# xyy7/Learning-based-RGB-D-Image-Compression

Measured on AMD Instinct MI355X. Metric: RGB-D Mpixels/s encode+decode, higher is better.
Workload: dtype f32; 1 GPU; c3_4x480x640; codec=ELIC_united ch4 q=2_2 (N=192,M=320), images_per_gpu=4, steps_per_call=4, images_per_call=16, calls=5, weights=synthetic seed 0 (stress recipe), streams=per image, y_bytes_last_batch=15943588, engine_instances=5, conv_tiles=throughput, warmup_steps_run=40, launch=HIP graph per call shape, pairs_in_flight=80

## Files before the change

include/rgbd_amd.h:

```cpp
#ifndef RGBD_AMD_H
#define RGBD_AMD_H

#include <stddef.h>
#include <stdint.h>

#ifdef __cplusplus
extern "C" {
#endif

#define RGBD_AMD_ABI_VERSION 1

int rgbd_abi_version(void);

int rgbd_set_blocking_sync(int32_t on);
int rgbd_get_blocking_sync(void);

int rgbd_pmf_to_quantized_cdf(const float* pmf, int32_t n, int32_t precision, uint32_t* cdf_out);

typedef struct rgbd_tables rgbd_tables;

int rgbd_tables_create(const int32_t* cdf, int32_t cdf_stride, const int32_t* cdf_sizes, const int32_t* offsets,
                       int32_t n_cdf, rgbd_tables** out);
void rgbd_tables_destroy(rgbd_tables* t);

// ... 157 lines not shown
int rgbd_elic_debug_floats(rgbd_elic* m, int32_t modality, float* x, float* scale, int64_t cap, int64_t* n);
int rgbd_elic_set_forced_symbols(rgbd_elic* m, int32_t modality, const int32_t* y_sym, int64_t n_y, const int32_t* z_sym,
                                 int64_t n_z);

int rgbd_debug_force_splitk(int32_t s);
int rgbd_debug_force_fuse(int32_t mode);
int rgbd_debug_force_subpix(int32_t mode);
int rgbd_debug_force_pair(int32_t mode);
int rgbd_elic_set_tile_mode(rgbd_elic* m, int32_t mode);
int rgbd_debug_bench_streams(int32_t n);
int rgbd_debug_force_blocked(int32_t on);
int rgbd_debug_force_ckbd(int32_t part);
int rgbd_debug_conv_log(int32_t on);
int64_t rgbd_debug_conv_log_read(char* buf, int64_t cap);
int rgbd_debug_force_tile(const char* cfg);
long rgbd_debug_tile_list(int32_t blocked, char* buf, long cap);
int rgbd_debug_tile_override(const char* csv);

int rgbd_pointwise_nchw(int32_t op, const float* x_dev, int32_t n, int32_t c, int32_t h, int32_t w, int32_t oh, int32_t ow,
                        const float* w0, const float* w1, float* y_dev, void* stream);

int rgbd_ref_channel_mean(const float* x_dev, int32_t n, int32_t c, int32_t h, int32_t w, float* mean_dev, int32_t mstride,
                          void* stream);
int rgbd_ref_linear(const float* weight, const float* x_dev, int32_t n, int32_t K, int32_t J, const int32_t* row_class, int32_t form,
                    int32_t act, int32_t stage, float* y_dev, void* stream);
int rgbd_ref_sigmoid_gate(const float* t_dev, const float* mul_dev, const float* res_dev, int32_t n, int32_t c, int32_t h, int32_t w,
                          int32_t per_image, int32_t threads, float* y_dev, void* stream);
int rgbd_ref_small_conv_nchw(const float* x_dev, int32_t n, int32_t cin, int32_t h, int32_t w, const float* weight, const float* bias,
                             int32_t cout, int32_t k, int32_t stride, int32_t pad, int32_t act, int32_t ckbd, const int32_t* kblocks,
                             int32_t nkblocks, const float* res1_dev, const float* mul_dev, const float* res2_dev, float* y_dev,
// ... 47 lines not shown
```

learning-based-rgb-d-image-compression_amd/_lib.py:

```python
import ctypes
import os
import subprocess

_HERE = os.path.dirname(os.path.abspath(__file__))
_SO = os.path.join(_HERE, "librgbd_amd.so")
_SO = os.environ.get("RGBD_AMD_LIB", _SO)
_SRCS = ["conv_mfma.hip", "conv_mfma_blk.hip", "pointwise.hip", "swin.hip", "entropy.hip", "metrics.hip", "coder_abi.hip", "gdn.hip", "engine.hip", "engine_abi.hip"]
_LIB = None

ERRORS = {-22: "invalid argument", -12: "out of memory", -5: "HIP runtime error", -28: "buffer too small",
          -1: "wrong call order / missing weights or tables"}


class RgbdError(RuntimeError):
    pass


def check(rc: int, what: str = ""):
    if rc != 0:
        raise RgbdError(f"librgbd_amd: {what} failed with {rc} ({ERRORS.get(rc, 'unknown')})")


class ConvFormsOps(ctypes.Structure):
    _fields_ = [("x_dev", ctypes.c_void_p)] + [(n, ctypes.POINTER(ctypes.c_float)) for n in
# ... 8 lines not shown
               [(n, ctypes.c_int32) for n in ("cout2", "act_mid", "cout3", "x_off", "x_total", "y_off", "y_total", "y2_off", "y2_total",
                                              "y3_off", "y3_total", "groups")] + \
               [("set", ConvFormsOps * 2)]


def build(force: bool = False, verbose: bool = False) -> str:
    from concurrent.futures import ThreadPoolExecutor

    csrc = os.path.join(_HERE, "csrc")
    objdir = os.path.join(csrc, "build")
    hdrs = [os.path.join(csrc, "common.h"), os.path.join(csrc, "exact_math.h"),
            os.path.join(os.path.dirname(_HERE), "include", "rgbd_amd.h")]
    body, tiles = os.path.join(csrc, "conv_mfma_body.h"), os.path.join(csrc, "conv_tiles.h")
    extra = {"conv_mfma.hip": [body, tiles, os.path.join(csrc, "tile_table.h"), os.path.join(csrc, "tile_table_loaded.h"),
                               os.path.join(csrc, "tile_table_blk.h"), os.path.join(csrc, "tile_table_blk_loaded.h")],
             "conv_mfma_blk.hip": [body, tiles]}
    hdrs.append(os.path.join(csrc, "splitk_table.h"))
    extra["coder_abi.hip"] = extra["gdn.hip"] = [os.path.join(csrc, "engine_internal.h")]
    extra["engine.hip"] = extra["engine_abi.hip"] = [os.path.join(csrc, "engine_internal.h"), os.path.join(csrc, "engine.h"),
                                                     os.path.join(csrc, "conv_args.h")]
    hipcc = os.environ.get("HIPCC", "/opt/rocm/bin/hipcc")
    os.makedirs(objdir, exist_ok=True)
    jobs, objs = [], []
    for name in _SRCS:
        src, obj = os.path.join(csrc, name), os.path.join(objdir, name + ".o")
        objs.append(obj)
        deps = [src] + hdrs + extra.get(name, [])
        if force or not os.path.exists(obj) or any(os.path.getmtime(obj) < os.path.getmtime(d) for d in deps):
            flags = ["-mllvm", "-amdgpu-mfma-vgpr-form"] if name == "conv_mfma_blk.hip" else []
            jobs.append([hipcc, "-O3", "--offload-arch=gfx950", "-ffp-contract=off", "-fPIC", "-std=c++17"] + flags + ["-c", src, "-o", obj])
    if not jobs and os.path.exists(_SO) and all(os.path.getmtime(_SO) >= os.path.getmtime(o) for o in objs):
        return _SO
    if verbose:
        for j in jobs:
            print(" ".join(j))
    with ThreadPoolExecutor(max_workers=4) as ex:
        list(ex.map(subprocess.check_call, jobs))
    subprocess.check_call([hipcc, "--offload-arch=gfx950", "-fPIC", "-shared"] + objs + ["-o", _SO])
    return _SO


def lib():
    global _LIB
    if _LIB is not None:
# ... 101 lines not shown
        "rgbd_debug_force_ckbd": (ctypes.c_int, [c_i32]),
        "rgbd_debug_force_blocked": (ctypes.c_int, [c_i32]),
        "rgbd_debug_force_fuse": (ctypes.c_int, [c_i32]),
        "rgbd_debug_force_subpix": (ctypes.c_int, [c_i32]),
        "rgbd_layernorm": (ctypes.c_int, [c_vp, c_i64, c_i32, c_i32, c_vp, c_vp, c_vp, c_i32, c_vp]),
        "rgbd_debug_force_layernorm_form": (None, [c_i32]),
        "rgbd_layernorm2": (ctypes.c_int, [c_vp, c_i64, c_i32, c_i32, c_vp, c_vp, c_vp, c_i32, c_vp, c_vp, c_vp, c_vp, c_vp]),
        "rgbd_window_attention": (ctypes.c_int, [c_vp] + [c_i32] * 7 + [c_vp, c_vp, c_i32, c_vp, c_vp, c_vp, c_vp]),
        "rgbd_patch_merge_gather": (ctypes.c_int, [c_vp] + [c_i32] * 5 + [c_vp, c_i32, c_vp]),
        "rgbd_pixel_shuffle2": (ctypes.c_int, [c_vp] + [c_i32] * 5 + [c_vp, c_i32, c_vp]),
        "rgbd_debug_force_pair": (ctypes.c_int, [c_i32]),
        "rgbd_debug_fail_captures": (ctypes.c_int, [c_i32]),
        "rgbd_debug_bench_streams": (ctypes.c_int, [c_i32]),
        "rgbd_elic_set_tile_mode": (ctypes.c_int, [ctypes.c_void_p, c_i32]),
        "rgbd_debug_force_tile": (ctypes.c_int, [ctypes.c_char_p]),
        "rgbd_debug_conv_log": (ctypes.c_int, [c_i32]),
        "rgbd_debug_conv_log_read": (c_i64, [ctypes.c_char_p, c_i64]),
        "rgbd_debug_tile_override": (ctypes.c_int, [ctypes.c_char_p]),
        "rgbd_debug_tile_list": (ctypes.c_long, [c_i32, ctypes.c_char_p, ctypes.c_long]),
        "rgbd_conv_bench": (ctypes.c_int, [c_i32] * 11 + [f32p]),
        "rgbd_elic_profile_dump": (ctypes.c_int, [c_vp, ctypes.c_char_p]),
        "rgbd_elic_profile_read": (ctypes.c_int, [c_vp, ctypes.POINTER(ctypes.c_double), i64p,
                                                  ctypes.POINTER(ctypes.c_double)]),
        "rgbd_elic_profile_read_executed": (ctypes.c_int, [c_vp, ctypes.POINTER(ctypes.c_double)]),
    }
    for name, (res, args) in sig.items():
        fn = getattr(L, name)
        fn.restype = res
        fn.argtypes = args
    _LIB = L
    return L


EXPORTS = ["rgbd_abi_version", "rgbd_set_blocking_sync", "rgbd_get_blocking_sync", "rgbd_pmf_to_quantized_cdf", "rgbd_tables_create", "rgbd_tables_destroy",
           "rgbd_rans_max_bytes", "rgbd_rans_encode", "rgbd_rans_decoder_create", "rgbd_rans_decoder_set_stream",
           "rgbd_rans_decoder_decode", "rgbd_rans_decoder_destroy", "rgbd_rans_encode_batch_dev", "rgbd_rans_decode_batch_dev", "rgbd_ckbd_quant_index", "rgbd_ckbd_dequant", "rgbd_conv2d_nchw", "rgbd_conv2d_ref_nchw", "rgbd_conv_forms_nchw", "rgbd_pointwise_nchw", "rgbd_ref_channel_mean", "rgbd_ref_linear", "rgbd_ref_sigmoid_gate",
           "rgbd_ref_small_conv_nchw", "rgbd_ref_deconv_s2_nchw", "rgbd_elic_create",
           "rgbd_elic_destroy", "rgbd_elic_set_ref_blocks", "rgbd_elic_get_refnum", "rgbd_elic_ref_table_misses", "rgbd_elic_clone_shared", "rgbd_elic_set_tensor", "rgbd_elic_set_tables", "rgbd_elic_set_scale_table",
           "rgbd_elic_finalize", "rgbd_elic_compress", "rgbd_elic_forward", "rgbd_elic_stream_count", "rgbd_elic_stream",
           "rgbd_elic_decompress", "rgbd_elic_create_r2d", "rgbd_elic_create_stf", "rgbd_elic_create_single", "rgbd_elic_compress_single", "rgbd_elic_decompress_single", "rgbd_elic_forward_single", "rgbd_elic_compress_united", "rgbd_elic_decompress_united", "rgbd_elic_debug_tensor", "rgbd_elic_debug_symbols", "rgbd_elic_set_debug_floats", "rgbd_elic_debug_floats", "rgbd_elic_set_forced_symbols", "rgbd_elic_set_profile", "rgbd_elic_graph_count", "rgbd_elic_workspace_bytes", "rgbd_msssim_workspace_bytes", "rgbd_msssim_stats", "rgbd_layernorm", "rgbd_debug_force_layernorm_form",
           "rgbd_layernorm2", "rgbd_window_attention", "rgbd_patch_merge_gather", "rgbd_pixel_shuffle2",
           "rgbd_elic_profile_read", "rgbd_elic_profile_read_executed", "rgbd_debug_force_splitk", "rgbd_debug_force_fuse", "rgbd_debug_force_subpix", "rgbd_debug_force_pair", "rgbd_debug_fail_captures", "rgbd_debug_force_ckbd", "rgbd_debug_force_blocked", "rgbd_debug_bench_streams", "rgbd_elic_set_tile_mode", "rgbd_debug_force_tile", "rgbd_debug_conv_log", "rgbd_debug_conv_log_read", "rgbd_debug_tile_override", "rgbd_debug_tile_list", "rgbd_conv_bench",
           "rgbd_elic_profile_dump", "rgbd_elic_create_stf_single", "rgbd_slice_quant_index", "rgbd_slice_dequant", "rgbd_lrp_update",
           "rgbd_ckbd_estimate_part", "rgbd_slice_estimate", "rgbd_ckbd_part", "rgbd_z_quant", "rgbd_z_dequant", "rgbd_eb_forward",
           "rgbd_elic_create_ckbd", "rgbd_gdn_nchw", "rgbd_gdn_parametrize", "rgbd_debug_force_gdn_tile", "rgbd_gdn_bench",
           "rgbd_guided_window_attention", "rgbd_aligner_create", "rgbd_aligner_forward", "rgbd_elic_decompress_single_mid",
           "rgbd_elic_forward_single_mid"]


_BS_HOLDERS = 0


def set_blocking_sync(on: bool) -> bool:
    global _BS_HOLDERS
    import gc

    L = lib()
# ... 9 lines not shown
```

learning-based-rgb-d-image-compression_amd/csrc/common.h:

```cpp
#pragma once
#include <hip/hip_runtime.h>
#include <stdint.h>
#include <stdio.h>

#define RGBD_OK 0
#define RGBD_EINVAL (-22)
#define RGBD_ENOMEM (-12)
#define RGBD_EHIP (-5)
#define RGBD_ENOSPC (-28)
#define RGBD_ESTATE (-1)

#define HIP_TRY(expr)                                                                          \
    do {                                                                                       \
        hipError_t _e = (expr);                                                                \
        if (_e != hipSuccess) {                                                                \
            fprintf(stderr, "[rgbd_amd] %s:%d %s -> %s\n", __FILE__, __LINE__, #expr,          \
                    hipGetErrorString(_e));                                                    \
            return RGBD_EHIP;                                                                  \
        }                                                                                      \
    } while (0)

struct Act {
    float* p = nullptr;
    int n = 0, h = 0, w = 0, c = 0, cs = 0;
// ... 103 lines not shown
    if (nphase == 1 && out_px_per_image <= 512) {
        if (taps_per_phase == 1) s = K >= 1500 ? 8 : (K >= 700 ? 4 : (K >= 350 ? 2 : 1));
        else s = K >= 5000 ? 8 : (K >= 1000 ? 4 : (K >= 500 ? 2 : 1));
    } else {
        s = (int)((K + 800) / 1600);
        if (s > 8) s = 8;
    }
    if (s > cin_pad / 16) s = cin_pad / 16;
    if (s < 1) s = 1;
    return s;
}

int launch_conv(const ConvArgs& a, hipStream_t s);
int conv_fused_plan(int cout_pad, int cout2_pad, int ntaps, int N, int GH, int GW, int loaded);
int launch_conv_fused(const ConvArgs& a, hipStream_t s);
int conv_log_enable(int on);
int conv_tile_override(const char* csv);
long conv_log_read(char* buf, long cap);
long conv_tile_list(int blocked, char* buf, long cap);

int launch_sigmoid_gate_ref(const float* t, int tcs, const float* mul, int mcs, const float* res2, int r2cs, float* y, int ycs,
                            int N, int HW, int C, int per_image, int threads, hipStream_t s);

int launch_nchw_to_nhwc16(const float* src, int N, int C, int H, int W, float* dst, int cs, hipStream_t s, int perm = 0);
int launch_nhwc_to_nchw_clamp(const float* src, int N, int C, int H, int W, int cs, float* dst, int clamp01,
                              hipStream_t s, int perm = 0);
int launch_maxpool7s3(const float* x, int N, int H, int W, int cs, float* y, int OH, int OW, hipStream_t s,
                      const float* x1 = nullptr, float* y1 = nullptr);
int launch_bilinear(const float* x, int N, int h, int w, int cs, float* y, int H, int W, hipStream_t s, const float* x1 = nullptr,
                    float* y1 = nullptr, int ref_channels = 0);
// ... 149 lines not shown
```

learning-based-rgb-d-image-compression_amd/csrc/conv_mfma.hip:

```cpp
#include <array>
#include <map>
#include <string>

#include "conv_mfma_body.h"
#include "conv_tiles.h"

bool conv_blk_tile_ok(int wm, int mt, int nt, int max_tiles);
int launch_conv_blk(const ConvArgs& a, const Choice& c, hipStream_t s);
int launch_conv_fused_blk(const ConvArgs& a, int cls, hipStream_t s);

namespace {

Choice choose(const ConvArgs& a, int max_tiles = 16)
{
    static const int cand[][3] = {{2, 3, 8}, {2, 2, 8}, {2, 5, 4}, {2, 4, 4}, {2, 3, 4}, {2, 2, 4}, {2, 1, 4}, {2, 5, 2}, {2, 4, 2},
                                  {2, 3, 2}, {2, 2, 2}, {2, 1, 2}, {2, 5, 1}, {2, 4, 1}, {2, 3, 1}, {2, 2, 1},
                                  {2, 1, 1}, {1, 3, 2}, {1, 2, 2}, {1, 1, 2}, {1, 3, 1}, {1, 2, 1}, {1, 1, 1}};
    int max_taps = 1;
    for (int p = 0; p < a.nphase; ++p) max_taps = a.taps.n[p] > max_taps ? a.taps.n[p] : max_taps;
    const double K = (double)max_taps * a.cin_pad / a.splitk;
    const int ck = a.ckbd ? 1 : 0;
    const int GWe = ck ? (a.GW + 1) / 2 : a.GW;
    Choice best{2, 4, 4, 16, 4, false};
    double best_cost = -1.0;
// ... 299 lines not shown
    }
    if (t) {
        c.wm = t->wm;
        c.mt = t->mt;
        c.nt = t->nt;
        set_mode(c, t->kc, t->dma);
        c.tw_log2 = pick_tw_log2(a.ckbd ? (a.GW + 1) / 2 : a.GW, a.GH, 16 * t->nt * (t->wm == 2 ? 2 : 4));
    }
    if (g_log_on) {
        char key[160];
        snprintf(key, sizeof(key), "%d,%d,%d,%d,%d,%d,%d,%d,%d", a.N * (a.groups == 2 ? 2 : 1), a.H, a.W, a.cin_pad, a.cout_pad, a.ntaps_total,
                 a.nphase > 1 ? a.OS : a.IS, a.nphase + 10 * a.ckbd + (a.blocked ? 100 : 0), a.splitk);
        std::lock_guard<std::mutex> lk(g_log_mu);
        ++g_log[key];
    }
    if (!g_ovr.empty()) {
        char key[160];
        snprintf(key, sizeof(key), "%d,%d,%d,%d,%d,%d,%d,%d,%d", a.N * (a.groups == 2 ? 2 : 1), a.H, a.W, a.cin_pad, a.cout_pad, a.ntaps_total,
                 a.nphase > 1 ? a.OS : a.IS, a.nphase + 10 * a.ckbd + (a.blocked ? 100 : 0), a.splitk);
        std::lock_guard<std::mutex> lk(g_log_mu);
        auto it = g_ovr.find(key);
        if (it != g_ovr.end()) {
            c.wm = it->second[0];
            c.mt = it->second[1];
            c.nt = it->second[2];
            set_mode(c, it->second[3], it->second[4]);
            c.tw_log2 = pick_tw_log2(a.ckbd ? (a.GW + 1) / 2 : a.GW, a.GH, 16 * c.nt * (c.wm == 2 ? 2 : 4));
        }
    }
    static const char* force_env = getenv("RGBD_CONV_FORCE");
    const char* force = g_conv_force[0] ? g_conv_force : force_env;
    if (force) {
        int wm = c.wm, mt = c.mt, nt = c.nt, kc = c.kc, dm = c.dma;
        sscanf(force, "%d,%d,%d,%d,%d", &wm, &mt, &nt, &kc, &dm);
        c.wm = wm;
        c.mt = mt;
        c.nt = nt;
        set_mode(c, kc, dm);
        c.tw_log2 = pick_tw_log2(a.ckbd ? (a.GW + 1) / 2 : a.GW, a.GH, 16 * nt * (wm == 2 ? 2 : 4));
    }
    static const bool debug = getenv("RGBD_CONV_DEBUG") != nullptr;
    if (debug)
        fprintf(stderr, "[conv] N=%d GH=%d GW=%d cin=%d cout=%d taps=%d IS=%d nph=%d -> WM=%d MT=%d NT=%d KC=%d tw=%d dma=%d\n", a.N,
                a.GH, a.GW, a.cin_pad, a.cout_pad, a.taps.n[0], a.IS, a.nphase, c.wm, c.mt, c.nt, c.kc, 1 << c.tw_log2, (int)c.dma);
    if (c.ring && !ring_ok(a)) return RGBD_ENOSPC;
    if (a.blocked) return launch_conv_blk(a, c, s);
    RGBD_TILES_MAIN_RING(RGBD_RING4)
    RGBD_TILES_MAIN_RING(RGBD_RING3)
    if (c.ring) return RGBD_ENOSPC;
    RGBD_TILES_MAIN(RGBD_CASE)
    return RGBD_EINVAL;
}

static const bool g_fuse_off = getenv("RGBD_NO_FUSE") != nullptr;
int g_fuse_force = -1;
int g_fuse_lead_off = 0;

int conv_fused_plan(int cout_pad, int cout2_pad, int ntaps, int N, int GH, int GW, int loaded)
{
// ... 46 lines not shown
```

learning-based-rgb-d-image-compression_amd/csrc/conv_mfma_body.h:

```cpp
#pragma once
#include <stdlib.h>
#include <string.h>

#include <algorithm>
#include <map>
#include <mutex>
#include <string>

#include "common.h"
#include "exact_math.h"

typedef float f32x4 __attribute__((ext_vector_type(4)));

__device__ __forceinline__ float sigmoid_f32(float x)
{
    return __builtin_amdgcn_rcpf(1.0f + __builtin_amdgcn_exp2f(x * -1.4426950408889634f));
}

template <int N>
__device__ __forceinline__ void rgbd_wait_vmcnt()
{
    asm volatile("s_waitcnt vmcnt(%0)" ::"n"(N) : "memory");
}

template <int WM, int WN, int MT, int NT, int KC, bool DMA, int G2, bool LEAD = false, int NB = 2, bool BLK = false>
__device__ __forceinline__ void conv_mfma_body(const ConvArgs& a, int tw_log2, int tiles_x, int tiles_y, int taps_per_stage,
                                               int tab_f)
{
    constexpr int TM = 16 * MT * WM;
    constexpr int TP = 16 * NT * WN;
    constexpr bool RING = NB > 2;
    static_assert(!RING || (DMA && KC == 16 && G2 == 0 && TP % 64 == 0), "ring staging: DMA, 16-channel stages, whole waves of patch slots");
    constexpr int RS = KC > 16 ? KC + 4 : KC;
    constexpr int C4 = KC / 4;
    constexpr int WR = 8;
    constexpr int PR = TP >= 128 ? 12 : (TP >= 64 ? 6 : 4);
    extern __shared__ __attribute__((aligned(16))) float smem[];
// ... 66 lines not shown
    f32x4 acc[MT][NT];
    f32x4 tot[BLK ? MT : 1][BLK ? NT : 1];
#pragma unroll
    for (int i = 0; i < MT; ++i) {
        f32x4 b4 = (f32x4){0.f, 0.f, 0.f, 0.f};
        const int cob = co0 + (wm * MT + i) * 16 + q * 4;
        if (a.bias_mode != 0 && cob < a.cout_pad) b4 = *reinterpret_cast<const f32x4*>(gbias + cob);
        const f32x4 z4 = (f32x4){0.f, 0.f, 0.f, 0.f};
#pragma unroll
        for (int j = 0; j < NT; ++j) {
            acc[i][j] = (a.bias_mode == 2 && split == 0) ? b4 : z4;
            if constexpr (BLK) tot[i][j] = a.bias_mode == 1 ? b4 : z4;
        }
    }
    auto fold = [&](int c16) {
        if constexpr (BLK) {
            if ((a.blk_end[c16 >> 5] >> (c16 & 31)) & 1u) {
                auto tie = [](f32x4& t, bool wait) {
                    float t0 = t[0], t1 = t[1], t2 = t[2], t3 = t[3];
                    if (wait) asm volatile("s_nop 11" : "+v"(t0), "+v"(t1), "+v"(t2), "+v"(t3));
                    else asm volatile("" : "+v"(t0), "+v"(t1), "+v"(t2), "+v"(t3));
                    t = (f32x4){t0, t1, t2, t3};
                };
                tie(acc[MT - 1][NT - 1], true);
                if constexpr (NT > 1) tie(acc[MT - 1][NT - 2], false);
                else if constexpr (MT > 1) tie(acc[MT - 2][NT - 1], false);
#pragma unroll
                for (int i = 0; i < MT; ++i)
#pragma unroll
                    for (int j = 0; j < NT; ++j) {
                        tot[i][j] += acc[i][j];
                        acc[i][j] = (f32x4){0.f, 0.f, 0.f, 0.f};
                    }
            }
        }
    };

    int ppy[NT], ppx[NT];
#pragma unroll
    for (int j = 0; j < NT; ++j) {
        const int p = (wn * NT + j) * 16 + l15;
        ppy[j] = p >> tw_log2;
        ppx[j] = p & (TW - 1);
        if (ck) ppx[j] = 2 * ppx[j] + (((ty0 + ppy[j]) & 1) ^ (a.ckbd == 1 ? 1 : 0));
    }

    const int npatch4 = PH * PW * C4;
    int brow0[NT];
#pragma unroll
    for (int j = 0; j < NT; ++j) brow0[j] = ((ppy[j] * a.IS) * PW + ppx[j] * a.IS) * RS + q * 4;
// ... 501 lines not shown
            int cbs[UB];
            bool ok[UB];
#pragma unroll
            for (int u = 0; u < UB; ++u) {
                const int f = tid + (u0 + u) * 256;
                const int p = f / S4, c4 = f - p * S4;
                const int wmc = c4 / (4 * EMT), ii = (c4 / 4) % EMT;
                const int cb = co0 + (wmc * MT + ip + ii) * 16 + (c4 & 3) * 4;
                const int gy = ty0 + (p >> tw_log2);
                const int gx = tx0 + (ck ? 2 * (p & (TW - 1)) + ((gy & 1) ^ (a.ckbd == 1 ? 1 : 0)) : (p & (TW - 1)));
                ok[u] = ip + ii < MT && cb < a.cout_store && gy < a.GH && gx < a.GW;
                cbs[u] = cb;
                const int oy = a.subpix ? ((cb >> 3) & 1) : oy_off, ox = a.subpix ? ((cb >> 2) & 1) : ox_off;
                pixs[u] = (unsigned)((gy * a.OS + oy) * a.OW + (gx * a.OS + ox));
                v[u] = *reinterpret_cast<const f32x4*>(smem + p * SW + c4 * 4);
                const f32x4 z = (f32x4){0.f, 0.f, 0.f, 0.f};
                r1[u] = (ok[u] && a.res1) ? *reinterpret_cast<const f32x4*>(r1n + (size_t)((pixs[u] * (unsigned)a.r1cs + cb) * 4u)) : z;
                ml[u] = (ok[u] && a.mul) ? *reinterpret_cast<const f32x4*>(mln + (size_t)((pixs[u] * (unsigned)a.mcs + cb) * 4u)) : z;
                r2[u] = (ok[u] && a.res2) ? *reinterpret_cast<const f32x4*>(r2n + (size_t)((pixs[u] * (unsigned)a.r2cs + cb) * 4u)) : z;
            }
#pragma unroll
            for (int u = 0; u < UB; ++u) {
                if (!ok[u]) continue;
                const int cb = cbs[u];
                f32x4 w = v[u];
                if (a.partial) {
                    *reinterpret_cast<f32x4*>(ptn + (size_t)((pixs[u] * (unsigned)a.cout_pad + cb) * 4u)) = w;
                    continue;
                }
                if (a.bias_mode == 0) w += *reinterpret_cast<const f32x4*>(gbias + cb);
                if (a.res1) w += r1[u];
                if (a.act == ACT_RELU) {
#pragma unroll
                    for (int e = 0; e < 4; ++e) w[e] = fmaxf(w[e], 0.f);
                } else if (a.act == ACT_LEAKY) {
#pragma unroll
                    for (int e = 0; e < 4; ++e) w[e] = w[e] > 0.f ? w[e] : w[e] * 0.01f;
                } else if (a.act == ACT_SIGMOID) {
#pragma unroll
                    for (int e = 0; e < 4; ++e) w[e] = a.exact_math ? rgbd_sigmoid_ref(w[e]) : sigmoid_f32(w[e]);
                }
                if (a.mul) w *= ml[u];
                if (a.res2) w += r2[u];
                *reinterpret_cast<f32x4*>(yn + (size_t)((pixs[u] * (unsigned)a.ycs + (a.subpix ? 0 : cb)) * 4u)) = w;
                if (a.y2) *reinterpret_cast<f32x4*>(y2n + (size_t)((pixs[u] * (unsigned)a.y2cs + cb) * 4u)) = w;
            }
        }
    }
}

template <int WM, int WN, int MT, int NT, int KC, bool DMA, int NB = 2, bool BLK = false>
__global__ __launch_bounds__(256) void conv_mfma_kernel(ConvArgs a, int tw_log2, int tiles_x, int tiles_y,
                                                         int taps_per_stage, int tab_f)
{
    conv_mfma_body<WM, WN, MT, NT, KC, DMA, 0, false, NB, BLK>(a, tw_log2, tiles_x, tiles_y, taps_per_stage, tab_f);
}

template <int WM, int WN, int MT, int NT, int KC, bool DMA, int G2, bool LEAD, bool BLK = false>
__global__ __launch_bounds__(256) __attribute__((amdgpu_waves_per_eu(2))) void conv_mfma_kernel_fused(
    ConvArgs a, int tw_log2, int tiles_x, int tiles_y, int taps_per_stage, int tab_f)
// ... 110 lines not shown
```

learning-based-rgb-d-image-compression_amd/csrc/engine_abi.hip:

```cpp
#include "engine.h"

extern "C" {

int rgbd_abi_version(void) { return RGBD_AMD_ABI_VERSION; }

static std::atomic<int> g_live_engines{0};
static std::mutex g_policy_mu;
static bool g_policy_done[64] = {false};

static int ensure_wait_policy()
{
    static const bool spin = getenv("RGBD_SPIN_WAIT") != nullptr;
    if (spin) return RGBD_OK;
    int dev = 0;
    HIP_TRY(hipGetDevice(&dev));
    std::lock_guard<std::mutex> g(g_policy_mu);
    if (dev < 0 || dev >= 64 || g_policy_done[dev]) return RGBD_OK;
    if (g_live_engines.load() == 0) {
        std::unique_lock<std::shared_mutex> cap_lk(g_capture_mu);
        HIP_TRY(hipDeviceSynchronize());
        HIP_TRY(hipSetDeviceFlags(hipDeviceScheduleBlockingSync));
    }
    g_policy_done[dev] = true;
    return RGBD_OK;
// ... 543 lines not shown
    if (!rc && e != hipSuccess) rc = RGBD_EHIP;
    for (int g = 0; g < G && !rc; ++g) {
        const FormsSet& f = fs[g];
        rc = guard_intact(f.y, ycs);
        if (!rc && f.y2) rc = guard_intact(f.y2, y2cs);
        if (!rc && f.y3) rc = guard_intact(f.y3, y3cs);
    }
    return rc;
}

int rgbd_debug_force_tile(const char* cfg)
{
    snprintf(g_conv_force, sizeof(g_conv_force), "%s", cfg ? cfg : "");
    ++g_cfg_epoch;
    return RGBD_OK;
}

int rgbd_debug_tile_override(const char* csv)
{
    ++g_cfg_epoch;
    return conv_tile_override(csv);
}

int rgbd_debug_conv_log(int32_t on) { return conv_log_enable(on); }
int64_t rgbd_debug_conv_log_read(char* buf, int64_t cap) { return conv_log_read(buf, (long)cap); }
long rgbd_debug_tile_list(int32_t blocked, char* buf, long cap) { return conv_tile_list(blocked, buf, cap); }

int rgbd_elic_set_tile_mode(rgbd_elic* m, int32_t mode)
{
    if (!m || mode < 0 || mode > 1) return RGBD_EINVAL;
// ... 897 lines not shown
```

Baseline: 19.24 Mpx/s.

## Add weight-stationary persistent 1x1 conv kernel for listed shapes

Adds a new persistent 1x1 convolution kernel that keeps the weight slab resident in LDS and streams pixel tiles through a 3-stage ring. Workgroups are sized to the CU count and loop over tiles. A shape table decides when the dispatcher uses it instead of the generic MFMA conv path, unless a tile config is pinned or an env var disables it. The epilogue is shared by factoring it into helpers. The aim is to stop reloading weights per tile for pointwise convs, at the cost of 160KB of LDS per workgroup and lower occupancy.

Measured after the change: 19.36 Mpx/s, median of 5. No clear change (+0.6%).

```diff
diff --git a/include/rgbd_amd.h b/include/rgbd_amd.h
--- a/include/rgbd_amd.h
+++ b/include/rgbd_amd.h
@@ -195,6 +195,7 @@
 int rgbd_debug_conv_log(int32_t on);
 int64_t rgbd_debug_conv_log_read(char* buf, int64_t cap);
 int rgbd_debug_force_tile(const char* cfg);
+int rgbd_debug_force_ws1x1(int32_t mode, int32_t max_workgroups);
 long rgbd_debug_tile_list(int32_t blocked, char* buf, long cap);
 int rgbd_debug_tile_override(const char* csv);
 
diff --git a/learning-based-rgb-d-image-compression_amd/_lib.py b/learning-based-rgb-d-image-compression_amd/_lib.py
--- a/learning-based-rgb-d-image-compression_amd/_lib.py
+++ b/learning-based-rgb-d-image-compression_amd/_lib.py
@@ -5,7 +5,7 @@
 _HERE = os.path.dirname(os.path.abspath(__file__))
 _SO = os.path.join(_HERE, "librgbd_amd.so")
 _SO = os.environ.get("RGBD_AMD_LIB", _SO)
-_SRCS = ["conv_mfma.hip", "conv_mfma_blk.hip", "pointwise.hip", "swin.hip", "entropy.hip", "metrics.hip", "coder_abi.hip", "gdn.hip", "engine.hip", "engine_abi.hip"]
+_SRCS = ["conv_mfma.hip", "conv_mfma_blk.hip", "conv_ws1x1.hip", "pointwise.hip", "swin.hip", "entropy.hip", "metrics.hip", "coder_abi.hip", "gdn.hip", "engine.hip", "engine_abi.hip"]
 _LIB = None
 
 ERRORS = {-22: "invalid argument", -12: "out of memory", -5: "HIP runtime error", -28: "buffer too small",
@@ -46,7 +46,9 @@
     body, tiles = os.path.join(csrc, "conv_mfma_body.h"), os.path.join(csrc, "conv_tiles.h")
     extra = {"conv_mfma.hip": [body, tiles, os.path.join(csrc, "tile_table.h"), os.path.join(csrc, "tile_table_loaded.h"),
                                os.path.join(csrc, "tile_table_blk.h"), os.path.join(csrc, "tile_table_blk_loaded.h")],
-             "conv_mfma_blk.hip": [body, tiles]}
+             "conv_mfma_blk.hip": [body, tiles],
+             "conv_ws1x1.hip": [body, os.path.join(csrc, "conv_ws1x1.h"), os.path.join(csrc, "ws1x1_table.h"),
+                                os.path.join(csrc, "ws1x1_table_loaded.h")]}
     hdrs.append(os.path.join(csrc, "splitk_table.h"))
     extra["coder_abi.hip"] = extra["gdn.hip"] = [os.path.join(csrc, "engine_internal.h")]
     extra["engine.hip"] = extra["engine_abi.hip"] = [os.path.join(csrc, "engine_internal.h"), os.path.join(csrc, "engine.h"),
@@ -59,7 +61,7 @@
         objs.append(obj)
         deps = [src] + hdrs + extra.get(name, [])
         if force or not os.path.exists(obj) or any(os.path.getmtime(obj) < os.path.getmtime(d) for d in deps):
-            flags = ["-mllvm", "-amdgpu-mfma-vgpr-form"] if name == "conv_mfma_blk.hip" else []
+            flags = ["-mllvm", "-amdgpu-mfma-vgpr-form"] if name in ("conv_mfma_blk.hip", "conv_ws1x1.hip") else []
             jobs.append([hipcc, "-O3", "--offload-arch=gfx950", "-ffp-contract=off", "-fPIC", "-std=c++17"] + flags + ["-c", src, "-o", obj])
     if not jobs and os.path.exists(_SO) and all(os.path.getmtime(_SO) >= os.path.getmtime(o) for o in objs):
         return _SO
@@ -191,6 +193,7 @@
         "rgbd_debug_bench_streams": (ctypes.c_int, [c_i32]),
         "rgbd_elic_set_tile_mode": (ctypes.c_int, [ctypes.c_void_p, c_i32]),
         "rgbd_debug_force_tile": (ctypes.c_int, [ctypes.c_char_p]),
+        "rgbd_debug_force_ws1x1": (ctypes.c_int, [c_i32, c_i32]),
         "rgbd_debug_conv_log": (ctypes.c_int, [c_i32]),
         "rgbd_debug_conv_log_read": (c_i64, [ctypes.c_char_p, c_i64]),
         "rgbd_debug_tile_override": (ctypes.c_int, [ctypes.c_char_p]),
@@ -217,7 +220,7 @@
            "rgbd_elic_finalize", "rgbd_elic_compress", "rgbd_elic_forward", "rgbd_elic_stream_count", "rgbd_elic_stream",
            "rgbd_elic_decompress", "rgbd_elic_create_r2d", "rgbd_elic_create_stf", "rgbd_elic_create_single", "rgbd_elic_compress_single", "rgbd_elic_decompress_single", "rgbd_elic_forward_single", "rgbd_elic_compress_united", "rgbd_elic_decompress_united", "rgbd_elic_debug_tensor", "rgbd_elic_debug_symbols", "rgbd_elic_set_debug_floats", "rgbd_elic_debug_floats", "rgbd_elic_set_forced_symbols", "rgbd_elic_set_profile", "rgbd_elic_graph_count", "rgbd_elic_workspace_bytes", "rgbd_msssim_workspace_bytes", "rgbd_msssim_stats", "rgbd_layernorm", "rgbd_debug_force_layernorm_form",
            "rgbd_layernorm2", "rgbd_window_attention", "rgbd_patch_merge_gather", "rgbd_pixel_shuffle2",
-           "rgbd_elic_profile_read", "rgbd_elic_profile_read_executed", "rgbd_debug_force_splitk", "rgbd_debug_force_fuse", "rgbd_debug_force_subpix", "rgbd_debug_force_pair", "rgbd_debug_fail_captures", "rgbd_debug_force_ckbd", "rgbd_debug_force_blocked", "rgbd_debug_bench_streams", "rgbd_elic_set_tile_mode", "rgbd_debug_force_tile", "rgbd_debug_conv_log", "rgbd_debug_conv_log_read", "rgbd_debug_tile_override", "rgbd_debug_tile_list", "rgbd_conv_bench",
+           "rgbd_elic_profile_read", "rgbd_elic_profile_read_executed", "rgbd_debug_force_splitk", "rgbd_debug_force_fuse", "rgbd_debug_force_subpix", "rgbd_debug_force_pair", "rgbd_debug_fail_captures", "rgbd_debug_force_ckbd", "rgbd_debug_force_blocked", "rgbd_debug_bench_streams", "rgbd_elic_set_tile_mode", "rgbd_debug_force_tile", "rgbd_debug_force_ws1x1", "rgbd_debug_conv_log", "rgbd_debug_conv_log_read", "rgbd_debug_tile_override", "rgbd_debug_tile_list", "rgbd_conv_bench",
            "rgbd_elic_profile_dump", "rgbd_elic_create_stf_single", "rgbd_slice_quant_index", "rgbd_slice_dequant", "rgbd_lrp_update",
            "rgbd_ckbd_estimate_part", "rgbd_slice_estimate", "rgbd_ckbd_part", "rgbd_z_quant", "rgbd_z_dequant", "rgbd_eb_forward",
            "rgbd_elic_create_ckbd", "rgbd_gdn_nchw", "rgbd_gdn_parametrize", "rgbd_debug_force_gdn_tile", "rgbd_gdn_bench",
diff --git a/learning-based-rgb-d-image-compression_amd/csrc/common.h b/learning-based-rgb-d-image-compression_amd/csrc/common.h
--- a/learning-based-rgb-d-image-compression_amd/csrc/common.h
+++ b/learning-based-rgb-d-image-compression_amd/csrc/common.h
@@ -141,6 +141,8 @@
 int launch_conv(const ConvArgs& a, hipStream_t s);
 int conv_fused_plan(int cout_pad, int cout2_pad, int ntaps, int N, int GH, int GW, int loaded);
 int launch_conv_fused(const ConvArgs& a, hipStream_t s);
+int conv_ws1x1_dispatch(const ConvArgs& a, bool pinned, hipStream_t s);
+int conv_ws1x1_force(int mode, int max_workgroups);
 int conv_log_enable(int on);
 int conv_tile_override(const char* csv);
 long conv_log_read(char* buf, long cap);
diff --git a/learning-based-rgb-d-image-compression_amd/csrc/conv_mfma.hip b/learning-based-rgb-d-image-compression_amd/csrc/conv_mfma.hip
--- a/learning-based-rgb-d-image-compression_amd/csrc/conv_mfma.hip
+++ b/learning-based-rgb-d-image-compression_amd/csrc/conv_mfma.hip
@@ -337,6 +337,7 @@
         std::lock_guard<std::mutex> lk(g_log_mu);
         ++g_log[key];
     }
+    bool pinned = false;
     if (!g_ovr.empty()) {
         char key[160];
         snprintf(key, sizeof(key), "%d,%d,%d,%d,%d,%d,%d,%d,%d", a.N * (a.groups == 2 ? 2 : 1), a.H, a.W, a.cin_pad, a.cout_pad, a.ntaps_total,
@@ -344,6 +345,7 @@
         std::lock_guard<std::mutex> lk(g_log_mu);
         auto it = g_ovr.find(key);
         if (it != g_ovr.end()) {
+            pinned = true;
             c.wm = it->second[0];
             c.mt = it->second[1];
             c.nt = it->second[2];
@@ -354,6 +356,7 @@
     static const char* force_env = getenv("RGBD_CONV_FORCE");
     const char* force = g_conv_force[0] ? g_conv_force : force_env;
     if (force) {
+        pinned = true;
         int wm = c.wm, mt = c.mt, nt = c.nt, kc = c.kc, dm = c.dma;
         sscanf(force, "%d,%d,%d,%d,%d", &wm, &mt, &nt, &kc, &dm);
         c.wm = wm;
@@ -366,6 +369,7 @@
     if (debug)
         fprintf(stderr, "[conv] N=%d GH=%d GW=%d cin=%d cout=%d taps=%d IS=%d nph=%d -> WM=%d MT=%d NT=%d KC=%d tw=%d dma=%d\n", a.N,
                 a.GH, a.GW, a.cin_pad, a.cout_pad, a.taps.n[0], a.IS, a.nphase, c.wm, c.mt, c.nt, c.kc, 1 << c.tw_log2, (int)c.dma);
+    if (const int ws = conv_ws1x1_dispatch(a, pinned, s); ws <= 0) return ws;
     if (c.ring && !ring_ok(a)) return RGBD_ENOSPC;
     if (a.blocked) return launch_conv_blk(a, c, s);
     RGBD_TILES_MAIN_RING(RGBD_RING4)
diff --git a/learning-based-rgb-d-image-compression_amd/csrc/conv_mfma_body.h b/learning-based-rgb-d-image-compression_amd/csrc/conv_mfma_body.h
--- a/learning-based-rgb-d-image-compression_amd/csrc/conv_mfma_body.h
+++ b/learning-based-rgb-d-image-compression_amd/csrc/conv_mfma_body.h
@@ -21,6 +21,62 @@
 __device__ __forceinline__ void rgbd_wait_vmcnt()
 {
     asm volatile("s_waitcnt vmcnt(%0)" ::"n"(N) : "memory");
+}
+
+
+template <int MT, int NT>
+__device__ __forceinline__ void conv_mfma_tie(f32x4 (&acc)[MT][NT])
+{
+    auto tie = [](f32x4& t, bool wait) {
+        float t0 = t[0], t1 = t[1], t2 = t[2], t3 = t[3];
+        if (wait) asm volatile("s_nop 11" : "+v"(t0), "+v"(t1), "+v"(t2), "+v"(t3));
+        else asm volatile("" : "+v"(t0), "+v"(t1), "+v"(t2), "+v"(t3));
+        t = (f32x4){t0, t1, t2, t3};
+    };
+    tie(acc[MT - 1][NT - 1], true);
+    if constexpr (NT > 1) tie(acc[MT - 1][NT - 2], false);
+    else if constexpr (MT > 1) tie(acc[MT - 2][NT - 1], false);
+}
+
+template <int MT, int NT>
+__device__ __forceinline__ void conv_blk_fold(const ConvArgs& a, int c16, f32x4 (&acc)[MT][NT], f32x4 (&tot)[MT][NT])
+{
+    if ((a.blk_end[c16 >> 5] >> (c16 & 31)) & 1u) {
+        conv_mfma_tie<MT, NT>(acc);
+#pragma unroll
+        for (int i = 0; i < MT; ++i)
+#pragma unroll
+            for (int j = 0; j < NT; ++j) {
+                tot[i][j] += acc[i][j];
+                acc[i][j] = (f32x4){0.f, 0.f, 0.f, 0.f};
+            }
+    }
+}
+
+__device__ __forceinline__ f32x4 conv_epi_operand(bool on, const char* base, unsigned pix, int cs, int cb)
+{
+    return on ? *reinterpret_cast<const f32x4*>(base + (size_t)((pix * (unsigned)cs + cb) * 4u)) : (f32x4){0.f, 0.f, 0.f, 0.f};
+}
+
+__device__ __forceinline__ void conv_epi_finish(const ConvArgs& a, f32x4 w, f32x4 bias4, f32x4 r1, f32x4 ml, f32x4 r2, int cb,
+                                                unsigned pix, char* yn, char* y2n)
+{
+    if (a.bias_mode == 0) w += bias4;
+    if (a.res1) w += r1;
+    if (a.act == ACT_RELU) {
+#pragma unroll
+        for (int e = 0; e < 4; ++e) w[e] = fmaxf(w[e], 0.f);
+    } else if (a.act == ACT_LEAKY) {
+#pragma unroll
+        for (int e = 0; e < 4; ++e) w[e] = w[e] > 0.f ? w[e] : w[e] * 0.01f;
+    } else if (a.act == ACT_SIGMOID) {
+#pragma unroll
+        for (int e = 0; e < 4; ++e) w[e] = a.exact_math ? rgbd_sigmoid_ref(w[e]) : sigmoid_f32(w[e]);
+    }
+    if (a.mul) w *= ml;
+    if (a.res2) w += r2;
+    *reinterpret_cast<f32x4*>(yn + (size_t)((pix * (unsigned)a.ycs + (a.subpix ? 0 : cb)) * 4u)) = w;
+    if (a.y2) *reinterpret_cast<f32x4*>(y2n + (size_t)((pix * (unsigned)a.y2cs + cb) * 4u)) = w;
 }
 
 template <int WM, int WN, int MT, int NT, int KC, bool DMA, int G2, bool LEAD = false, int NB = 2, bool BLK = false>
@@ -117,26 +173,7 @@
         }
     }
     auto fold = [&](int c16) {
-        if constexpr (BLK) {
-            if ((a.blk_end[c16 >> 5] >> (c16 & 31)) & 1u) {
-                auto tie = [](f32x4& t, bool wait) {
-                    float t0 = t[0], t1 = t[1], t2 = t[2], t3 = t[3];
-                    if (wait) asm volatile("s_nop 11" : "+v"(t0), "+v"(t1), "+v"(t2), "+v"(t3));
-                    else asm volatile("" : "+v"(t0), "+v"(t1), "+v"(t2), "+v"(t3));
-                    t = (f32x4){t0, t1, t2, t3};
-                };
-                tie(acc[MT - 1][NT - 1], true);
-                if constexpr (NT > 1) tie(acc[MT - 1][NT - 2], false);
-                else if constexpr (MT > 1) tie(acc[MT - 2][NT - 1], false);
-#pragma unroll
-                for (int i = 0; i < MT; ++i)
-#pragma unroll
-                    for (int j = 0; j < NT; ++j) {
-                        tot[i][j] += acc[i][j];
-                        acc[i][j] = (f32x4){0.f, 0.f, 0.f, 0.f};
-                    }
-            }
-        }
+        if constexpr (BLK) conv_blk_fold<MT, NT>(a, c16, acc, tot);
     };
 
     int ppy[NT], ppx[NT];
@@ -668,10 +705,9 @@
                 const int oy = a.subpix ? ((cb >> 3) & 1) : oy_off, ox = a.subpix ? ((cb >> 2) & 1) : ox_off;
                 pixs[u] = (unsigned)((gy * a.OS + oy) * a.OW + (gx * a.OS + ox));
                 v[u] = *reinterpret_cast<const f32x4*>(smem + p * SW + c4 * 4);
-                const f32x4 z = (f32x4){0.f, 0.f, 0.f, 0.f};
-                r1[u] = (ok[u] && a.res1) ? *reinterpret_cast<const f32x4*>(r1n + (size_t)((pixs[u] * (unsigned)a.r1cs + cb) * 4u)) : z;
-                ml[u] = (ok[u] && a.mul) ? *reinterpret_cast<const f32x4*>(mln + (size_t)((pixs[u] * (unsigned)a.mcs + cb) * 4u)) : z;
-                r2[u] = (ok[u] && a.res2) ? *reinterpret_cast<const f32x4*>(r2n + (size_t)((pixs[u] * (unsigned)a.r2cs + cb) * 4u)) : z;
+                r1[u] = conv_epi_operand(ok[u] && a.res1, r1n, pixs[u], a.r1cs, cb);
+                ml[u] = conv_epi_operand(ok[u] && a.mul, mln, pixs[u], a.mcs, cb);
+                r2[u] = conv_epi_operand(ok[u] && a.res2, r2n, pixs[u], a.r2cs, cb);
             }
 #pragma unroll
             for (int u = 0; u < UB; ++u) {
@@ -682,22 +718,8 @@
                     *reinterpret_cast<f32x4*>(ptn + (size_t)((pixs[u] * (unsigned)a.cout_pad + cb) * 4u)) = w;
                     continue;
                 }
-                if (a.bias_mode == 0) w += *reinterpret_cast<const f32x4*>(gbias + cb);
-                if (a.res1) w += r1[u];
-                if (a.act == ACT_RELU) {
-#pragma unroll
-                    for (int e = 0; e < 4; ++e) w[e] = fmaxf(w[e], 0.f);
-                } else if (a.act == ACT_LEAKY) {
-#pragma unroll
-                    for (int e = 0; e < 4; ++e) w[e] = w[e] > 0.f ? w[e] : w[e] * 0.01f;
-                } else if (a.act == ACT_SIGMOID) {
-#pragma unroll
-                    for (int e = 0; e < 4; ++e) w[e] = a.exact_math ? rgbd_sigmoid_ref(w[e]) : sigmoid_f32(w[e]);
-                }
-                if (a.mul) w *= ml[u];
-                if (a.res2) w += r2[u];
-                *reinterpret_cast<f32x4*>(yn + (size_t)((pixs[u] * (unsigned)a.ycs + (a.subpix ? 0 : cb)) * 4u)) = w;
-                if (a.y2) *reinterpret_cast<f32x4*>(y2n + (size_t)((pixs[u] * (unsigned)a.y2cs + cb) * 4u)) = w;
+                const f32x4 bias4 = a.bias_mode == 0 ? *reinterpret_cast<const f32x4*>(gbias + cb) : (f32x4){0.f, 0.f, 0.f, 0.f};
+                conv_epi_finish(a, w, bias4, r1[u], ml[u], r2[u], cb, pixs[u], yn, y2n);
             }
         }
     }
diff --git a/learning-based-rgb-d-image-compression_amd/csrc/conv_ws1x1.h b/learning-based-rgb-d-image-compression_amd/csrc/conv_ws1x1.h
--- /dev/null
+++ b/learning-based-rgb-d-image-compression_amd/csrc/conv_ws1x1.h
@@ -0,0 +1,227 @@
+#pragma once
+#include "conv_mfma_body.h"
+
+constexpr int WS_WAVES = 8;
+constexpr int WS_NT = 2;
+constexpr int WS_NB = 3;
+constexpr int WS_WPIX = 16 * WS_NT;
+constexpr int WS_TP = WS_WAVES * WS_WPIX;
+constexpr int WS_STAGE_F = WS_WPIX * 16;
+constexpr int WS_EMT = 2;
+constexpr int WS_SW = 16 * WS_EMT + 4;
+constexpr int WS_RING_F = WS_NB * WS_STAGE_F;
+constexpr int WS_EPI_F = WS_WPIX * WS_SW;
+constexpr int WS_LDS_BYTES = 160 * 1024;
+constexpr int WS_SLAB_MAX = WS_LDS_BYTES - WS_WAVES * (WS_RING_F + WS_EPI_F) * 4;
+
+template <int N>
+__device__ __forceinline__ void ws_wait_vmcnt()
+{
+    static_assert(N >= 0 && N < 16, "vmcnt low bits");
+    __builtin_amdgcn_s_waitcnt(0x0F70 | N);
+    asm volatile("" ::: "memory");
+}
+
+template <int MT>
+__device__ __forceinline__ void ws_read_frags(f32x4 (&af)[MT], f32x4 (&bf)[WS_NT], const float* w, const float* p);
+template <>
+__device__ __forceinline__ void ws_read_frags<6>(f32x4 (&af)[6], f32x4 (&bf)[WS_NT], const float* w, const float* p)
+{
+    const unsigned wa = (unsigned)(size_t)w, pa = (unsigned)(size_t)p;
+    asm volatile(
+        "ds_read_b128 %0, %8\n\tds_read_b128 %6, %9\n\tds_read_b128 %7, %9 offset:1024\n\tds_read_b128 %1, %8 offset:1024\n\t"
+        "ds_read_b128 %2, %8 offset:2048\n\tds_read_b128 %3, %8 offset:3072\n\tds_read_b128 %4, %8 offset:4096\n\t"
+        "ds_read_b128 %5, %8 offset:5120\n\ts_waitcnt lgkmcnt(0)"
+        : "=&v"(af[0]), "=&v"(af[1]), "=&v"(af[2]), "=&v"(af[3]), "=&v"(af[4]), "=&v"(af[5]), "=&v"(bf[0]), "=&v"(bf[1])
+        : "v"(wa), "v"(pa)
+        : "memory");
+}
+template <>
+__device__ __forceinline__ void ws_read_frags<3>(f32x4 (&af)[3], f32x4 (&bf)[WS_NT], const float* w, const float* p)
+{
+    const unsigned wa = (unsigned)(size_t)w, pa = (unsigned)(size_t)p;
+    asm volatile(
+        "ds_read_b128 %0, %5\n\tds_read_b128 %3, %6\n\tds_read_b128 %4, %6 offset:1024\n\tds_read_b128 %1, %5 offset:1024\n\t"
+        "ds_read_b128 %2, %5 offset:2048\n\ts_waitcnt lgkmcnt(0)"
+        : "=&v"(af[0]), "=&v"(af[1]), "=&v"(af[2]), "=&v"(bf[0]), "=&v"(bf[1])
+        : "v"(wa), "v"(pa)
+        : "memory");
+}
+
+template <int MT, bool BLK>
+__global__ __launch_bounds__(64 * WS_WAVES) void conv_ws1x1_kernel(ConvArgs a, int ntiles, int npix)
+{
+    constexpr int TM = 16 * MT, NT = WS_NT;
+    extern __shared__ __attribute__((aligned(16))) float smem[];
+    const int tid = threadIdx.x;
+    const int lane = tid & 63;
+    const int wave = __builtin_amdgcn_readfirstlane(tid >> 6);
+    const int l15 = lane & 15, q = lane >> 4;
+    const int n16 = a.cin_pad / 16;
+    const int co0 = blockIdx.y * TM;
+    const bool g1 = blockIdx.z != 0;
+    const float* const gx = g1 ? a.g1.x : a.x;
+    const float* const gw = g1 ? a.g1.w : a.w;
+    const float* const gbias = g1 ? a.g1.bias : a.bias;
+    float* const gy = g1 ? a.g1.y : a.y;
+    const float* const gres1 = g1 ? a.g1.res1 : a.res1;
+    const float* const gmul = g1 ? a.g1.mul : a.mul;
+    const float* const gres2 = g1 ? a.g1.res2 : a.res2;
+    float* const gy2 = g1 ? a.g1.y2 : a.y2;
+
+    float* const slab = smem;
+    float* const ring = smem + n16 * TM * 16 + wave * WS_RING_F;
+    float* const est = smem + n16 * TM * 16 + WS_WAVES * WS_RING_F + wave * WS_EPI_F;
+
+    const int sw = (4 - ((lane >> 4) & 3)) & 3;
+    {
+        const int r = lane >> 2;
+        const int cq = (lane & 3) ^ sw;
+        const size_t wrow = (size_t)a.ntaps_total * a.cin_pad;
+        const int tapw = (int)a.taps.wt[0][0] * a.cin_pad;
+        for (int i = wave; i < n16 * MT; i += WS_WAVES) {
+            const int c = i / MT, mt = i - c * MT;
+            const int co = co0 + mt * 16 + r;
+            const float* src = gw + (size_t)(co < a.cout_pad ? co : co0) * wrow + tapw + c * 16 + cq * 4;
+            __builtin_amdgcn_global_load_lds((const __attribute__((address_space(1))) void*)src,
+                                             (__attribute__((address_space(3))) void*)(slab + (c * TM + mt * 16) * 16), 16, 0, 0);
+        }
+    }
+
+    const int G = gridDim.x, b = blockIdx.x;
+    const int ntl = b < ntiles ? (ntiles - b + G - 1) / G : 0;
+    const int S = __builtin_amdgcn_readfirstlane(ntl * n16);
+    int ic = 0, it = b, ibuf = 0, left = S;
+    const float *isrc0 = gx, *isrc1 = gx;
+    auto set_src = [&](int t) {
+        const int p0 = t * WS_TP + wave * WS_WPIX + (lane >> 2);
+        const int cq = (lane & 3) ^ sw;
+        isrc0 = gx + (size_t)min(p0, npix - 1) * a.xcs + cq * 4;
+        isrc1 = gx + (size_t)min(p0 + 16, npix - 1) * a.xcs + cq * 4;
+    };
+    auto issue = [&]() {
+        float* dst = ring + ibuf * WS_STAGE_F;
+        __builtin_amdgcn_global_load_lds((const __attribute__((address_space(1))) void*)(isrc0 + ic * 16),
+                                         (__attribute__((address_space(3))) void*)dst, 16, 0, 0);
+        __builtin_amdgcn_global_load_lds((const __attribute__((address_space(1))) void*)(isrc1 + ic * 16),
+                                         (__attribute__((address_space(3))) void*)(dst + 256), 16, 0, 0);
+        ibuf = ibuf == WS_NB - 1 ? 0 : ibuf + 1;
+        --left;
+        if (++ic == n16) {
+            ic = 0;
+            it += G;
+            if (left > 0) set_src(it);
+        }
+    };
+    if (left > 0) set_src(it);
+#pragma unroll
+    for (int st = 0; st < WS_NB - 1; ++st)
+        if (left > 0) issue();
+    f32x4 b4[MT];
+#pragma unroll
+    for (int i = 0; i < MT; ++i) {
+        const int cob = co0 + i * 16 + q * 4;
+        b4[i] = (f32x4){0.f, 0.f, 0.f, 0.f};
+        if (a.bias_mode != 0 && cob < a.cout_pad) b4[i] = *reinterpret_cast<const f32x4*>(gbias + cob);
+    }
+    f32x4 be[(MT + WS_EMT - 1) / WS_EMT];
+#pragma unroll
+    for (int ip = 0; ip < MT; ip += WS_EMT) {
+        const int i = ip + ((lane % (4 * WS_EMT)) >> 2);
+        const int cb = co0 + i * 16 + (lane & 3) * 4;
+        be[ip / WS_EMT] = (f32x4){0.f, 0.f, 0.f, 0.f};
+        if (a.bias_mode == 0 && i < MT && cb < a.cout_pad) be[ip / WS_EMT] = *reinterpret_cast<const f32x4*>(gbias + cb);
+    }
+    ws_wait_vmcnt<0>();
+    asm volatile("s_barrier" ::: "memory");
+
+    const int qs = (q ^ ((4 - (l15 >> 2)) & 3)) * 4;
+    int cbuf = 0, gst = 0;
+    for (int k = 0; k < ntl; ++k) {
+        const int t = b + k * G;
+        f32x4 acc[MT][NT];
+        f32x4 tot[BLK ? MT : 1][BLK ? NT : 1];
+        const f32x4 z4 = (f32x4){0.f, 0.f, 0.f, 0.f};
+#pragma unroll
+        for (int i = 0; i < MT; ++i)
+#pragma unroll
+            for (int j = 0; j < NT; ++j) {
+                acc[i][j] = a.bias_mode == 2 ? b4[i] : z4;
+                if constexpr (BLK) tot[i][j] = a.bias_mode == 1 ? b4[i] : z4;
+            }
+        for (int c = 0; c < n16; ++c, ++gst) {
+            if (gst + 1 < S) ws_wait_vmcnt<(WS_NB - 2) * 2>();
+            else ws_wait_vmcnt<0>();
+            if (left > 0) issue();
+            const float* cur_w = slab + c * TM * 16;
+            const float* cur_p = ring + cbuf * WS_STAGE_F;
+            f32x4 af[MT], bf[NT];
+            ws_read_frags<MT>(af, bf, cur_w + l15 * 16 + qs, cur_p + l15 * 16 + qs);
+#pragma unroll
+            for (int e = 0; e < 4; ++e)
+#pragma unroll
+                for (int i = 0; i < MT; ++i)
+#pragma unroll
+                    for (int j = 0; j < NT; ++j)
+                        acc[i][j] = __builtin_amdgcn_mfma_f32_16x16x4f32(af[i][e], bf[j][e], acc[i][j], 0, 0, 0);
+            if constexpr (BLK) conv_blk_fold<MT, NT>(a, c, acc, tot);
+            cbuf = cbuf == WS_NB - 1 ? 0 : cbuf + 1;
+        }
+        conv_mfma_tie<MT, NT>(acc);
+        if constexpr (BLK) {
+#pragma unroll
+            for (int i = 0; i < MT; ++i)
+#pragma unroll
+                for (int j = 0; j < NT; ++j) acc[i][j] = tot[i][j] + acc[i][j];
+        }
+
+        const int p0 = t * WS_TP + wave * WS_WPIX;
+        if (p0 >= npix) continue;
+        char* yn = reinterpret_cast<char*>(gy + (size_t)p0 * a.ycs);
+        const char* r1n = reinterpret_cast<const char*>(gres1 + (size_t)p0 * a.r1cs);
+        const char* mln = reinterpret_cast<const char*>(gmul + (size_t)p0 * a.mcs);
+        const char* r2n = reinterpret_cast<const char*>(gres2 + (size_t)p0 * a.r2cs);
+        char* y2n = reinterpret_cast<char*>(gy2 + (size_t)p0 * a.y2cs);
+        for (int ip = 0; ip < MT; ip += WS_EMT) {
+            f32x4 bias4 = be[0];
+#pragma unroll
+            for (int e = 1; e < (MT + WS_EMT - 1) / WS_EMT; ++e)
+                if (ip == e * WS_EMT) bias4 = be[e];
+            asm volatile("s_waitcnt lgkmcnt(0)" ::: "memory");
+#pragma unroll
+            for (int j = 0; j < NT; ++j)
+#pragma unroll
+                for (int i = 0; i < MT; ++i)
+                    if (i >= ip && i < ip + WS_EMT)
+                        *reinterpret_cast<f32x4*>(est + (j * 16 + l15) * WS_SW + (i - ip) * 16 + q * 4) = acc[i][j];
+            asm volatile("s_waitcnt lgkmcnt(0)" ::: "memory");
+            constexpr int S4 = 4 * WS_EMT;
+            constexpr int EU = WS_WPIX * S4 / 64;
+            f32x4 r1[EU], ml[EU], r2[EU], v[EU];
+            unsigned pixs[EU];
+            int cbs[EU];
+            bool ok[EU];
+#pragma unroll
+            for (int u = 0; u < EU; ++u) {
+                const int f = lane + u * 64;
+                const int p = f / S4, c4 = f - p * S4;
+                const int ii = c4 >> 2;
+                const int cb = co0 + (ip + ii) * 16 + (c4 & 3) * 4;
+                ok[u] = ip + ii < MT && cb < a.cout_store && p0 + p < npix;
+                cbs[u] = cb;
+                pixs[u] = (unsigned)p;
+                v[u] = *reinterpret_cast<const f32x4*>(est + p * WS_SW + c4 * 4);
+                r1[u] = conv_epi_operand(ok[u] && a.res1, r1n, pixs[u], a.r1cs, cb);
+                ml[u] = conv_epi_operand(ok[u] && a.mul, mln, pixs[u], a.mcs, cb);
+                r2[u] = conv_epi_operand(ok[u] && a.res2, r2n, pixs[u], a.r2cs, cb);
+            }
+#pragma unroll
+            for (int u = 0; u < EU; ++u) asm volatile("" ::"v"(r1[u]), "v"(ml[u]), "v"(r2[u]));
+#pragma unroll
+            for (int u = 0; u < EU; ++u) {
+                if (!ok[u]) continue;
+                conv_epi_finish(a, v[u], bias4, r1[u], ml[u], r2[u], cbs[u], pixs[u], yn, y2n);
+            }
+        }
+    }
+}
diff --git a/learning-based-rgb-d-image-compression_amd/csrc/conv_ws1x1.hip b/learning-based-rgb-d-image-compression_amd/csrc/conv_ws1x1.hip
--- /dev/null
+++ b/learning-based-rgb-d-image-compression_amd/csrc/conv_ws1x1.hip
@@ -0,0 +1,110 @@
+#include <atomic>
+
+#include "conv_ws1x1.h"
+
+namespace {
+
+std::atomic<int> g_ws_mode{-1};
+std::atomic<int> g_ws_maxwg{0};
+
+struct WsShape {
+    int N, H, W, cin_pad, cout_pad, blocked;
+};
+const WsShape kWs[] = {
+#include "ws1x1_table.h"
+    {0, 0, 0, 0, 0, 0}};
+const WsShape kWsLoaded[] = {
+#include "ws1x1_table_loaded.h"
+    {0, 0, 0, 0, 0, 0}};
+
+bool ws_listed(const ConvArgs& a)
+{
+    const int aN = a.N * (a.groups == 2 ? 2 : 1);
+    for (const WsShape* t = a.loaded ? kWsLoaded : kWs; t->N; ++t)
+        if (t->N == aN && t->H == a.H && t->W == a.W && t->cin_pad == a.cin_pad && t->cout_pad == a.cout_pad &&
+            t->blocked == (a.blocked ? 1 : 0))
+            return true;
+    return false;
+}
+
+int ws_mt(const ConvArgs& a)
+{
+    if (!ring_ok(a) || a.splitk > 1 || a.partial || a.subpix || a.w2 || a.w3) return 0;
+    if (a.min_dy || a.min_dx || a.OS != 1 || a.OH != a.H || a.OW != a.W || a.GH != a.OH || a.GW != a.OW) return 0;
+    if ((long)a.N * a.OH * a.OW >= ((long)1 << 31) - 2 * WS_TP) return 0;
+    if (a.cin_pad % 16 || a.cin_pad / 16 > 256) return 0;
+    const long row = (long)a.cin_pad * 4;
+    if (a.cout_pad > 48 && 96 * row <= WS_SLAB_MAX) return 6;
+    if (48 * row <= WS_SLAB_MAX) return 3;
+    return 0;
+}
+
+int ws_cu_count(int dev, int* out)
+{
+    static std::mutex mu;
+    static int cus[64] = {0};
+    std::lock_guard<std::mutex> lk(mu);
+    if (dev >= 0 && dev < 64 && cus[dev] > 0) {
+        *out = cus[dev];
+        return RGBD_OK;
+    }
+    int n = 0;
+    HIP_TRY(hipDeviceGetAttribute(&n, hipDeviceAttributeMultiprocessorCount, dev));
+    if (n < 1) n = 1;
+    if (dev >= 0 && dev < 64) cus[dev] = n;
+    *out = n;
+    return RGBD_OK;
+}
+
+template <int MT, bool BLK>
+int ws_launch(const ConvArgs& a, int max_wg, hipStream_t s)
+{
+    constexpr int TM = 16 * MT;
+    const size_t lds = (size_t)TM * a.cin_pad * 4 + (size_t)WS_WAVES * (WS_RING_F + WS_EPI_F) * 4;
+    if (lds > (size_t)WS_LDS_BYTES) return RGBD_ENOSPC;
+    void (*kern)(ConvArgs, int, int) = conv_ws1x1_kernel<MT, BLK>;
+    int dev = 0;
+    HIP_TRY(hipGetDevice(&dev));
+    {
+        static std::mutex mu;
+        static bool configured[64] = {false};
+        std::lock_guard<std::mutex> lk(mu);
+        if (dev < 0 || dev >= 64 || !configured[dev]) {
+            HIP_TRY(hipFuncSetAttribute(reinterpret_cast<const void*>(kern), hipFuncAttributeMaxDynamicSharedMemorySize, WS_LDS_BYTES));
+            if (dev >= 0 && dev < 64) configured[dev] = true;
+        }
+    }
+    int cus = 1;
+    if (const int rc = ws_cu_count(dev, &cus)) return rc;
+    const int npix = a.N * a.OH * a.OW;
+    const int ntiles = (npix + WS_TP - 1) / WS_TP;
+    const int ycount = (a.cout_pad + TM - 1) / TM, sets = a.groups == 2 ? 2 : 1;
+    int G = std::max(1, cus / (ycount * sets));
+    G = max_wg > 0 ? std::min(G, max_wg) : std::min(G, ntiles);
+    hipLaunchKernelGGL(kern, dim3((unsigned)G, (unsigned)ycount, (unsigned)sets), dim3(64 * WS_WAVES), lds, s, a, ntiles, npix);
+    HIP_TRY(hipGetLastError());
+    return RGBD_OK;
+}
+
+}
+
+int conv_ws1x1_force(int mode, int max_workgroups)
+{
+    if (mode < -1 || mode > 2 || max_workgroups < 0) return RGBD_EINVAL;
+    g_ws_mode = mode;
+    g_ws_maxwg = max_workgroups;
+    return RGBD_OK;
+}
+
+int conv_ws1x1_dispatch(const ConvArgs& a, bool pinned, hipStream_t s)
+{
+    static const bool off = getenv("RGBD_NO_WS1X1") != nullptr;
+    const int mode = g_ws_mode;
+    if (pinned || mode == 0 || (off && mode < 1)) return 1;
+    const int mt = ws_mt(a);
+    if (mode == 1 && !mt) return RGBD_ENOSPC;
+    if (!mt || (mode == -1 && !ws_listed(a))) return 1;
+    const int mw = g_ws_maxwg;
+    if (a.blocked) return mt == 6 ? ws_launch<6, true>(a, mw, s) : ws_launch<3, true>(a, mw, s);
+    return mt == 6 ? ws_launch<6, false>(a, mw, s) : ws_launch<3, false>(a, mw, s);
+}
diff --git a/learning-based-rgb-d-image-compression_amd/csrc/engine_abi.hip b/learning-based-rgb-d-image-compression_amd/csrc/engine_abi.hip
--- a/learning-based-rgb-d-image-compression_amd/csrc/engine_abi.hip
+++ b/learning-based-rgb-d-image-compression_amd/csrc/engine_abi.hip
@@ -581,6 +581,13 @@
     snprintf(g_conv_force, sizeof(g_conv_force), "%s", cfg ? cfg : "");
     ++g_cfg_epoch;
     return RGBD_OK;
+}
+
+int rgbd_debug_force_ws1x1(int32_t mode, int32_t max_workgroups)
+{
+    const int rc = conv_ws1x1_force(mode, max_workgroups);
+    if (!rc) ++g_cfg_epoch;
+    return rc;
 }
 
 int rgbd_debug_tile_override(const char* csv)
diff --git a/learning-based-rgb-d-image-compression_amd/csrc/ws1x1_table.h b/learning-based-rgb-d-image-compression_amd/csrc/ws1x1_table.h
--- /dev/null
+++ b/learning-based-rgb-d-image-compression_amd/csrc/ws1x1_table.h
@@ -0,0 +1,20 @@
+{1, 256, 320, 32, 192, 0},
+{1, 256, 320, 80, 192, 0},
+{2, 128, 160, 48, 48, 0},
+{2, 256, 320, 48, 48, 0},
+{2, 256, 320, 48, 192, 0},
+{2, 256, 320, 192, 192, 1},
+{16, 256, 320, 32, 192, 0},
+{16, 256, 320, 80, 192, 0},
+{32, 64, 80, 48, 192, 0},
+{32, 64, 80, 192, 192, 1},
+{32, 128, 160, 48, 48, 0},
+{32, 128, 160, 48, 192, 0},
+{32, 128, 160, 192, 48, 1},
+{32, 128, 160, 192, 96, 1},
+{32, 128, 160, 192, 192, 1},
+{32, 256, 320, 48, 48, 0},
+{32, 256, 320, 48, 192, 0},
+{32, 256, 320, 192, 48, 1},
+{32, 256, 320, 192, 96, 1},
+{32, 256, 320, 192, 192, 1},
diff --git a/learning-based-rgb-d-image-compression_amd/csrc/ws1x1_table_loaded.h b/learning-based-rgb-d-image-compression_amd/csrc/ws1x1_table_loaded.h
--- /dev/null
+++ b/learning-based-rgb-d-image-compression_amd/csrc/ws1x1_table_loaded.h
@@ -0,0 +1,15 @@
+{16, 256, 320, 32, 192, 0},
+{16, 256, 320, 80, 192, 0},
+{32, 64, 80, 48, 48, 0},
+{32, 64, 80, 48, 192, 0},
+{32, 64, 80, 192, 96, 1},
+{32, 128, 160, 48, 48, 0},
+{32, 128, 160, 48, 192, 0},
+{32, 128, 160, 192, 48, 1},
+{32, 128, 160, 192, 96, 1},
+{32, 128, 160, 192, 192, 1},
+{32, 256, 320, 48, 48, 0},
+{32, 256, 320, 48, 192, 0},
+{32, 256, 320, 192, 48, 1},
+{32, 256, 320, 192, 96, 1},
+{32, 256, 320, 192, 192, 1},
```
